# CederGroupHub/chgnet

Measured on NVIDIA H100. Metric: structures_per_sec_EFS, higher is better.
Workload: dtype f32

## Files before the change

chgnet_b200/_lib.py:

```python
from __future__ import annotations

import ctypes
import os
from ctypes import c_char_p, c_double, c_float, c_int32, c_int64, c_void_p

import torch
from torch import Tensor

_HERE = os.path.dirname(os.path.abspath(__file__))
LIB_PATH = os.path.join(_HERE, "libchgnet_b200.so")

P, I, F, D, I64 = c_void_p, c_int32, c_float, c_double, c_int64

SIGNATURES: dict[str, list] = {
    "chg_embed_atoms": [P, P, I, P, P],
    "chg_edge_geometry": [P, P, P, P, P, P, I, P, P, P, P],
    "chg_bond_basis_embed": [P, P, I, P, P, I, F, F, I, P, P, P, P, P, P],
    "chg_bond_basis_bwd": [P, P, I, P, P, I, F, F, I, P, P, P, P, P, P, P],
    "chg_angle_basis_embed": [P, P, P, I, P, I, P, P, P, P],
    "chg_angle_basis_bwd": [P, P, P, I, P, I, P, P, P, P, P],
    "chg_linear": [P, P, I, I, P, P, P, P, I, P, P],
    "chg_gather_rows": [P, P, I, I, P, P],
    "chg_scatter_rows": [P, P, I, I, P, P],
    "chg_atom_conv_fwd": [P, P, P, P, P, P, I, P, P, P, P, P, P, P],
    "chg_atom_conv_bwd": [P, P, P, P, P, P, I, P, P, P, P, P, P, P, P, P],
    "chg_segment_sum": [P, I, P, P, I, I, I, P, I, P],
    "chg_atom_conv_fused": [P, P, P, P, P, P, P, I, I, P, P, P, P, P, P, P],
    "chg_bond_conv_fused": [P, P, P, P, P, P, P, P, I, I, P, P, P, P, P, P, P, P],
    "chg_bond_conv_fwd": [P, P, P, P, P, P, P, I, P, P, P, P, P, P, P],
    "chg_bond_conv_bwd": [P, P, P, P, P, I, P, P, P, P, P, P, P, P, P],
    "chg_angle_update_fwd": [P, P, P, P, P, P, P, I, P, P, P, P],
    "chg_angle_update_bwd": [P, P, I, P, P, P, P],
    "chg_readout": [P, P, P, I, P, P, P, P, I, P, F, P, P, P, P, P, P, P],
    "chg_magmom": [P, I, P, F, P, P],
    "chg_force_virial": [P, P, P, P, P, P, P, P, P, P, I, P, P, P],
    "chg_wgrad": [P, P, I, P, I, P, I, P, I, I, P, I, P, P, P],
    "chg_colsum": [P, I, P, I, P, I, I, P, P],
    "chg_readout_bwd": [P, I, P, P, P, P, I, P, P, P, P, P, P, P, P],
    "chg_magmom_bwd": [P, I, P, F, P, P, P, P],
    "chg_loss_terms": [P, P, I, I, F, P, P, P],
    "chg_adam_step": [P, P, P, P, I64, F, F, F, F, F, I, P],
    "chg_edge_tangent": [P, P, P, P, P, P, P, P, I, P, P, P],
    "chg_bond_basis_tangent": [P, P, P, I, P, P, I, F, F, I, P, P, P, P, P, P],
    "chg_bond_basis_bwd2": [P, P, P, I, P, P, I, F, F, I, P, P, P, P, P, P],
    "chg_angle_basis_tangent": [P, P, P, P, I, P, I, P, P, P, P],
    "chg_angle_basis_bwd2": [P, P, P, P, I, P, I, P, P, P, P],
    "chg_atom_conv_tan": [P, P, P, P, P, P, P, I, P, P, P, P, P, P, P, P],
    "chg_atom_conv_bwd2": [P, P, P, P, P, P, P, P, P, I, P, P, P, P, P, P, P, P, P],
    "chg_bond_conv_tan": [P, P, P, P, P, P, P, P, I, P, P, P, P, P, P, P, P],
    "chg_bond_conv_bwd2": [P, P, P, P, P, P, P, P, P, I, P, P, P, P, P, P, P, P, P, P],
    "chg_angle_update_tan": [P, P, P, P, P, P, P, I, P, P, P, P, P],
    "chg_angle_update_bwd2": [P, P, P, P, I, P, P, P, P],
    "chg_readout_bwd2": [P, P, I, P, P, P, P, I, P, P, P, P, P, P, P, P, P, P, P, P],
    "chg_bond_basis_hvp": [P, P, P, I, P, P, I, F, F, I, P, P, P, P, P, P],
    "chg_angle_basis_hvp": [P, P, P, P, I, P, I, P, P, P, P],
    "chg_edge_tangent_bwd": [P, P, P, P, P, P, P, P, P, P, I, P, P],
    "chg_edge_tangent_bwd_virial": [P, P, P, P, P, P, P, P, P, P, P, P, I, P, P, P],
    "chg_dynamical_matrices": [P, P, P, P, P, I, I, P, I, P, P],
    "chg_dynamical_matrix_derivatives": [P, P, P, P, P, I, I, P, I, P, P, P],
# ... 141 lines not shown

    def atom_conv_bwd(self, pcn, pe, wag, center, nbr, d2u, save_p, g_agg, w2, ln, g_pre, g_w, g_p=None, g_ln=None):
        self._chk(pcn, pe, wag, center, nbr, d2u, save_p, g_agg, w2, ln, g_pre, g_w, g_p, g_ln)
        self._call("chg_atom_conv_bwd", _p(pcn), _p(pe), _p(wag), _p(center), _p(nbr), _p(d2u), center.shape[0],
                   _p(save_p), _p(g_agg), _p(w2), _p(ln), _p(g_pre), _p(g_w), _p(g_p), _p(g_ln))

    def _fused_work(self, n_rows: int, device) -> Tensor:
        need = int(self.lib.chg_gated_fused_workspace_floats(int(n_rows)))
        ws = getattr(self, "_fws", None)
        if ws is None or ws.device != device or ws.numel() < need:
            ws = torch.empty(need, dtype=torch.float32, device=device)
            self._fws = ws
        return ws

    def atom_conv_fused(self, pcn, pe, wag, center, nbr, d2u, ptr_c, w2t, b2, ln, agg, save_p):
        self._chk(pcn, pe, wag, center, nbr, d2u, ptr_c, w2t, b2, ln, agg, save_p)
        self._call("chg_atom_conv_fused", _p(pcn), _p(pe), _p(wag), _p(center), _p(nbr), _p(d2u), _p(ptr_c), center.shape[0],
                   agg.shape[0], _p(w2t), _p(b2), _p(ln), _p(agg), _p(save_p), _p(self._fused_work(center.shape[0], agg.device)))

    def bond_conv_fused(self, pij, px, pa, wbg, ang_atom, ang_i, ang_j, ptr_i, w2t, b2, ln, agg, save_pre, save_p):
        self._chk(pij, px, pa, wbg, ang_atom, ang_i, ang_j, ptr_i, w2t, b2, ln, agg, save_pre, save_p)
        self._call("chg_bond_conv_fused", _p(pij), _p(px), _p(pa), _p(wbg), _p(ang_atom), _p(ang_i), _p(ang_j), _p(ptr_i),
                   ang_i.shape[0], agg.shape[0], _p(w2t), _p(b2), _p(ln), _p(agg), _p(save_pre), _p(save_p),
                   _p(self._fused_work(ang_i.shape[0], agg.device)))

    def segment_sum(self, data, perm, ptr, accumulate, out):
        self._chk(data, perm, ptr)
        if not out.is_cuda or out.stride(1) != 1:
            raise ChgnetB200Error("segment_sum output must be a CUDA tensor with unit column stride")
        n_items = data.shape[0] if perm is None else perm.shape[0]
        self._call("chg_segment_sum", _p(data), data.shape[1], _p(perm), _p(ptr), ptr.shape[0] - 1, n_items,
                   int(accumulate), _p(out), out.stride(0))

    def bond_conv_fwd(self, pij, px, pa, wbg, ang_atom, ang_i, ang_j, w2t, b2, ln, upd, save_pre, save_p):
        self._chk(pij, px, pa, wbg, ang_atom, ang_i, ang_j, w2t, b2, ln, upd, save_pre, save_p)
        self._call("chg_bond_conv_fwd", _p(pij), _p(px), _p(pa), _p(wbg), _p(ang_atom), _p(ang_i), _p(ang_j),
                   ang_i.shape[0], _p(w2t), _p(b2), _p(ln), _p(upd), _p(save_pre), _p(save_p))

    def bond_conv_bwd(self, save_pre, save_p, wbg, ang_i, ang_j, g_agg, w2, ln, g_pre, gw_i, gw_j, g_p=None,
                      g_ln=None):
        self._chk(save_pre, save_p, wbg, ang_i, ang_j, g_agg, w2, ln, g_pre, gw_i, gw_j, g_p, g_ln)
        self._call("chg_bond_conv_bwd", _p(save_pre), _p(save_p), _p(wbg), _p(ang_i), _p(ang_j), ang_i.shape[0],
                   _p(g_agg), _p(w2), _p(ln), _p(g_pre), _p(gw_i), _p(gw_j), _p(g_p), _p(g_ln))

    def angle_update_fwd(self, pij, px, pa, ang, ang_atom, ang_i, ang_j, ln, ang_new, save_p):
        self._chk(pij, px, pa, ang, ang_atom, ang_i, ang_j, ln, ang_new, save_p)
        self._call("chg_angle_update_fwd", _p(pij), _p(px), _p(pa), _p(ang), _p(ang_atom), _p(ang_i), _p(ang_j),
                   ang_i.shape[0], _p(ln), _p(ang_new), _p(save_p))

    def angle_update_bwd(self, save_p, g_ang_in, ln, g_pre, g_ln=None):
        self._chk(save_p, g_ang_in, ln, g_pre, g_ln)
        self._call("chg_angle_update_bwd", _p(save_p), _p(g_ang_in), save_p.shape[0], _p(ln), _p(g_pre), _p(g_ln))

    @staticmethod
    def _chk_rows(*tensors: Tensor | None) -> None:
        for t in tensors:
            if t is not None and (not t.is_cuda or t.stride(-1) != 1):
                raise ChgnetB200Error("kernel arguments must be CUDA tensors with unit column stride")

    def _workspace(self, n_out: int, device) -> Tensor:
        ws = getattr(self, "_ws", None)
        if ws is None or ws.device != device:
            need = max(int(self.lib.chg_wgrad_workspace_floats(n)) for n in (64, 128, 256))
            ws = torch.empty(need, dtype=torch.float32, device=device)
            self._ws = ws
        return ws
# ... 225 lines not shown
```

chgnet_b200/csrc/common.cuh:

```cuda
#pragma once
#include <cuda_runtime.h>
#include <stdint.h>

#include "../../include/chgnet_b200.h"

namespace chg {

void set_error(const char* fmt, ...);
void count_launch();
int sm_count();
int linear_impl();
int gated_impl();
int segsum_unroll();
int segsum_force_s();

#define CHG_CHECK_ARG(cond, msg)                \
  do {                                          \
    if (!(cond)) {                              \
      chg::set_error("%s: %s", __func__, msg);  \
      return CHG_ERR_ARG;                       \
    }                                           \
  } while (0)

#define CHG_CUDA(expr)                                                              \
  do {                                                                              \
    cudaError_t _e = (expr);                                                        \
    if (_e != cudaSuccess) {                                                        \
      chg::set_error("%s: %s failed: %s", __func__, #expr, cudaGetErrorString(_e)); \
      return CHG_ERR_CUDA;                                                          \
    }                                                                               \
  } while (0)

#define CHG_LAUNCH_END()                                                            \
  do {                                                                              \
    cudaError_t _e = cudaGetLastError();                                            \
    if (_e != cudaSuccess) {                                                        \
      chg::set_error("%s: launch failed: %s", __func__, cudaGetErrorString(_e));    \
      return CHG_ERR_CUDA;                                                          \
    }                                                                               \
    chg::count_launch();                                                            \
    return CHG_OK;                                                                  \
  } while (0)

static inline cudaStream_t as_stream(void* s) { return reinterpret_cast<cudaStream_t>(s); }

#ifdef __CUDACC__

// ... 53 lines not shown
```

chgnet_b200/csrc/linear_ws.cu:

```cuda
#include <cuda.h>

#include "common.cuh"
#include "tc.cuh"

namespace chg {
namespace {

constexpr int NTHR = 288;
constexpr int PRODUCER_WARP = 8;
constexpr int S_IN = 2;
constexpr int PANEL = 128 * 128;
constexpr int IN_STAGE = 2 * PANEL;

struct Bars {
  uint64_t in_full[S_IN], in_empty[S_IN];
  uint64_t res_full, out_empty;
};

__device__ __forceinline__ void tma_load_2d(void* smem_dst, const CUtensorMap* map, int c0, int c1, uint64_t* bar) {
  asm volatile(
      "cp.async.bulk.tensor.2d.shared::cluster.global.mbarrier::complete_tx::bytes [%0], [%1, {%3, %4}], [%2];" ::"r"(
          tc::smem_u32(smem_dst)),
      "l"(map), "r"(tc::smem_u32(bar)), "r"(c0), "r"(c1)
      : "memory");
}
__device__ __forceinline__ void tma_store_2d(const CUtensorMap* map, int c0, int c1, const void* smem_src) {
  asm volatile("cp.async.bulk.tensor.2d.global.shared::cta.bulk_group [%0, {%2, %3}], [%1];" ::"l"(map),
               "r"(tc::smem_u32(smem_src)), "r"(c0), "r"(c1)
               : "memory");
}
__device__ __forceinline__ int swz(int r, int c) { return r * 128 + ((c ^ (r & 7)) << 4); }
__device__ __forceinline__ int panel_offset(int r, int col) { return (col >> 5) * PANEL + swz(r, (col & 31) >> 2) + (col & 3) * 4; }

template <int NT>
__global__ void __launch_bounds__(NTHR, 1)
linear_ws_kernel(const __grid_constant__ CUtensorMap map_x, const __grid_constant__ CUtensorMap map_y,
                 const __grid_constant__ CUtensorMap map_r, int m, int k, const float* __restrict__ wt,
                 const float* __restrict__ bias, int has_residual, int n_out) {
  extern __shared__ __align__(1024) uint8_t smem_raw[];
  uint8_t* s_in = smem_raw + ((1024u - (tc::smem_u32(smem_raw) & 1023u)) & 1023u);
  uint8_t* s_out = s_in + S_IN * IN_STAGE;
  uint8_t* s_bhi = s_out + (NT / 32) * PANEL;
  uint8_t* s_blo = s_bhi + (size_t)NT * k * 4;
  __shared__ __align__(8) Bars bars;
  __shared__ __align__(16) float s_bias[NT];

  const int tid = threadIdx.x, warp = tid >> 5, lane = tid & 31;
  const int col_base = blockIdx.y * NT;
  const int n_tiles = (m + 127) / 128;
  const int k_chunks = k / 64;

  {
    const int n4 = NT / 4, total4 = n4 * k;
    for (int i4 = tid; i4 < total4; i4 += NTHR) {
      const int kk = i4 / n4, n0 = (i4 % n4) * 4;
      const float4 v = ldg4(wt + (size_t)kk * n_out + col_base + n0);
#pragma unroll
      for (int e = 0; e < 4; ++e) {
        uint32_t hi, lo;
        tc::split_tf32(f4at(v, e), hi, lo);
        const uint32_t off = tc::kmajor_offset(n0 + e, kk, k);
        *reinterpret_cast<uint32_t*>(s_bhi + off) = hi;
        *reinterpret_cast<uint32_t*>(s_blo + off) = lo;
      }
    }
  }
  if (tid < NT) s_bias[tid] = bias != nullptr ? bias[col_base + tid] : 0.f;
  if (tid == 0) {
    for (int i = 0; i < S_IN; ++i) {
      tc::mbar_init(&bars.in_full[i], 1);
      tc::mbar_init(&bars.in_empty[i], 256);
    }
    tc::mbar_init(&bars.res_full, 1);
    tc::mbar_init(&bars.out_empty, 1);
    tc::mbar_fence_init();
  }
  tc::fence_async_smem();
  __syncthreads();

  if (warp == PRODUCER_WARP) {
    if (lane == 0) {
      int it = 0, tile_it = 0;
      for (int tile = blockIdx.x; tile < n_tiles; tile += gridDim.x, ++tile_it) {
        const int base = tile * 128;
        for (int kc = 0; kc < k_chunks; ++kc, ++it) {
          const int s = it % S_IN;
          tc::mbar_wait(&bars.in_empty[s], ((it / S_IN) & 1) ^ 1);
          tc::mbar_expect_tx(&bars.in_full[s], IN_STAGE);
          tma_load_2d(s_in + s * IN_STAGE, &map_x, kc * 64, base, &bars.in_full[s]);
          tma_load_2d(s_in + s * IN_STAGE + PANEL, &map_x, kc * 64 + 32, base, &bars.in_full[s]);
        }
        if (has_residual) {
          tc::mbar_wait(&bars.out_empty, (tile_it & 1) ^ 1);
          tc::mbar_expect_tx(&bars.res_full, (uint32_t)(NT / 32) * PANEL);
#pragma unroll
          for (int p = 0; p < NT / 32; ++p) tma_load_2d(s_out + p * PANEL, &map_r, col_base + p * 32, base, &bars.res_full);
        }
      }
    }
  } else {
    const int t = tid;
    const int row0 = (warp >> 2) * 64;
    const uint32_t bhi_addr = tc::smem_u32(s_bhi), blo_addr = tc::smem_u32(s_blo);
    const uint32_t sbo = (uint32_t)(k / 4) * 128;
    int it = 0, tile_it = 0;
    for (int tile = blockIdx.x; tile < n_tiles; tile += gridDim.x, ++tile_it) {
      const int base = tile * 128;
      float acc[NT / 2];
#pragma unroll
      for (int i = 0; i < NT / 2; ++i) acc[i] = 0.f;
      for (int kc = 0; kc < k_chunks; ++kc, ++it) {
        const int s = it % S_IN;
        tc::mbar_wait(&bars.in_full[s], (it / S_IN) & 1);
        const uint8_t* stage = s_in + s * IN_STAGE;
        tc::wg_gemm_k64<NT>(acc, [&](int r, int kk) { return *reinterpret_cast<const float*>(stage + panel_offset(row0 + r, kk)); },
                            bhi_addr + kc * 2048, blo_addr + kc * 2048, sbo);
        tc::mbar_arrive(&bars.in_empty[s]);
      }
      if (has_residual) tc::mbar_wait(&bars.res_full, tile_it & 1);
      tc::wg_barrier(2, 256);
#pragma unroll
      for (int i = 0; i < NT / 2; i += 2) {
        const int r = row0 + tc::frag_row(i), col = tc::frag_col(i);
        float2* dst = reinterpret_cast<float2*>(s_out + panel_offset(r, col));
        float2 o = make_float2(acc[i] + s_bias[col], acc[i + 1] + s_bias[col + 1]);
        if (has_residual) {
          const float2 res = *dst;
          o.x += res.x;
          o.y += res.y;
        }
        *dst = o;
      }
      tc::fence_async_smem();
// ... 10 lines not shown
  }
}

typedef CUresult (*EncodeFn)(CUtensorMap*, CUtensorMapDataType, cuuint32_t, void*, const cuuint64_t*,
                             const cuuint64_t*, const cuuint32_t*, const cuuint32_t*, CUtensorMapInterleave,
                             CUtensorMapSwizzle, CUtensorMapL2promotion, CUtensorMapFloatOOBfill);

EncodeFn encode_fn() {
  static EncodeFn fn = nullptr;
  static bool tried = false;
  if (!tried) {
    tried = true;
    void* p = nullptr;
    cudaDriverEntryPointQueryResult qres;
    if (cudaGetDriverEntryPoint("cuTensorMapEncodeTiled", &p, cudaEnableDefault, &qres) == cudaSuccess &&
        qres == cudaDriverEntryPointSuccess)
      fn = reinterpret_cast<EncodeFn>(p);
  }
  return fn;
}

bool make_map(CUtensorMap* map, const float* ptr, int rows, int cols) {
  EncodeFn fn = encode_fn();
  if (fn == nullptr) return false;
  const cuuint64_t dims[2] = {(cuuint64_t)cols, (cuuint64_t)rows};
  const cuuint64_t strides[1] = {(cuuint64_t)cols * 4};
  const cuuint32_t box[2] = {32, 128};
  const cuuint32_t estr[2] = {1, 1};
  return fn(map, CU_TENSOR_MAP_DATA_TYPE_FLOAT32, 2, const_cast<float*>(ptr), dims, strides, box, estr,
            CU_TENSOR_MAP_INTERLEAVE_NONE, CU_TENSOR_MAP_SWIZZLE_128B, CU_TENSOR_MAP_L2_PROMOTION_L2_128B,
            CU_TENSOR_MAP_FLOAT_OOB_FILL_NONE) == CUDA_SUCCESS;
}

template <int NT>
int launch_ws(const CUtensorMap& mx, const CUtensorMap& my, const CUtensorMap& mr, int m, int k, const float* wt,
              const float* bias, int has_residual, int n_out, cudaStream_t stream) {
  const int smem = S_IN * IN_STAGE + (NT / 32) * PANEL + 2 * NT * k * 4 + 1024;
  static int max_smem_set = 0;
  if (smem > max_smem_set) {
    CHG_CUDA(cudaFuncSetAttribute(linear_ws_kernel<NT>, cudaFuncAttributeMaxDynamicSharedMemorySize, smem));
    max_smem_set = smem;
  }
  const int n_tiles = (m + 127) / 128;
  const int col_tiles = n_out / NT;
  dim3 grid(min(n_tiles, max(1, sm_count() / col_tiles)), col_tiles);
  linear_ws_kernel<NT><<<grid, NTHR, smem, stream>>>(mx, my, mr, m, k, wt, bias, has_residual, n_out);
  CHG_LAUNCH_END();
}

}

int linear_ws(const float* x, int m, int k, const float* wt, const float* bias, const float* residual, int n_out,
              float* y, cudaStream_t stream) {
  if (k != 64 && k != 128) return 1;
  CUtensorMap mx, my, mr;
  if (!make_map(&mx, x, m, k) || !make_map(&my, y, m, n_out)) return 1;
  if (residual != nullptr) {
    if (!make_map(&mr, residual, m, n_out)) return 1;
  } else {
    mr = my;
  }
  if (n_out % 128 == 0 && k == 64) return launch_ws<128>(mx, my, mr, m, k, wt, bias, residual != nullptr, n_out, stream);
  return launch_ws<64>(mx, my, mr, m, k, wt, bias, residual != nullptr, n_out, stream);
}

}
```

chgnet_b200/csrc/native_engine.cu:

```cuda
#include <cstdarg>
#include <cstdio>
#include <cstring>
#include <string>

#include "common.cuh"

namespace chg {
namespace {

constexpr size_t ALIGN = 256;
constexpr int64_t PAD = 16;

struct GatedW {
  const float *w2t = nullptr, *w2 = nullptr, *b2 = nullptr, *ln = nullptr;
  const float *a_t = nullptr, *b_t = nullptr, *c_t = nullptr, *bias1 = nullptr;
  const float *a_b = nullptr, *b_b = nullptr, *c_b = nullptr;
  const float *wo_t = nullptr, *wo = nullptr, *bo = nullptr;
};
struct Weights {
  const float *emb, *freq_ag, *freq_bg, *freq_ang, *w3t, *w3, *wang_t, *wang;
  GatedW atom[CHG_MAX_CONV], bond[CHG_MAX_CONV], angle[CHG_MAX_CONV];
  const float *readout_ln, *mlp_wt, *mlp_w, *mlp_b, *w_last, *w_mag, *atom_ref;
};

// ... 251 lines not shown
    float* xn = c.f(true, (size_t)N * 64);
    atom_conv(n_conv - 1, x, xn);
    x = xn;
  }

  float* h_out = o.crystal_fea != nullptr ? c.f(false, (size_t)N * 64) : nullptr;
  float* g_x = grad ? c.f(true, (size_t)N * 64) : nullptr;
  c.zero(o.energy, (size_t)B * 8);
  c.zero(o.e_ref, (size_t)B * 8);
  RUN(c, "readout", chg_readout(x, b.z, b.owner, N, W.readout_ln, W.mlp_wt, W.mlp_w, W.mlp_b, hp.n_readout_hidden, W.w_last,
                                hp.b_last, W.atom_ref, o.site_e, h_out, o.energy, o.e_ref, g_x, st));
  if (o.crystal_fea != nullptr) seg(h_out, 64, nullptr, b.graph_ptr, B, N, 0, o.crystal_fea, 64);
  c.ar.reset_tmp();
  if (!grad) return c.rc;

  float* g_e = c.f(true, (size_t)Eu * 64);
  bool g_e_live = false;
  float* g_wag = c.f(true, (size_t)Eu * 64);
  c.zero(g_wag, (size_t)Eu * 256);
  float* g_wbg = has_ang ? c.f(true, (size_t)Es * 64) : nullptr;
  if (has_ang) c.zero(g_wbg, (size_t)Es * 256);
  float* g_a = has_ang ? c.f(true, (size_t)A * 64) : nullptr;
  bool g_a_live = false;

  auto atom_bwd = [&](int t) {
    const GatedW& g = W.atom[t];
    float* g_agg = c.f(false, (size_t)N * 64);
    lin(g_x, nullptr, N, 64, g.wo, nullptr, nullptr, nullptr, 64, g_agg);
    float* g_pre = c.f(false, (size_t)Ed * 128);
    float* g_w = c.f(false, (size_t)Ed * 64);
    RUN(c, "atom_conv_bwd", chg_atom_conv_bwd(sa[t].pcn, sa[t].pe, wag, b.center, b.nbr, b.d2u, Ed, sa[t].p, g_agg, g.w2, g.ln,
                                              g_pre, g_w, nullptr, nullptr, st));
    float* sp = c.f(false, (size_t)N * 256);
    seg(g_pre, 128, nullptr, b.ptr_c, N, Ed, 0, sp, 256);
    seg(g_pre, 128, b.perm_n, b.ptr_n, N, Ed, 0, sp + 128, 256);
    lin(sp, nullptr, N, 256, g.a_b, nullptr, g_x, nullptr, 64, g_x);
    float* spe = c.f(false, (size_t)Eu * 128);
    seg(g_pre, 128, b.perm_u, b.ptr_u, Eu, Ed, 0, spe, 128);
    lin(spe, nullptr, Eu, 128, g.b_b, nullptr, g_e_live ? g_e : nullptr, nullptr, 64, g_e);
    g_e_live = true;
    seg(g_w, 64, b.perm_u, b.ptr_u, Eu, Ed, 1, g_wag, 64);
    c.ar.reset_tmp();
  };
  auto angle_scatter = [&](const float* g_pre, const GatedW& g) {
    float* sp = c.f(false, (size_t)Es * 256);
    seg(g_pre, 128, nullptr, b.ptr_is, Es, A, 0, sp, 256);
    seg(g_pre, 128, b.perm_js, b.ptr_js, Es, A, 0, sp + 128, 256);
    lin(sp, nullptr, Es, 256, g.a_b, nullptr, g_e, b.short_ids, 64, g_e);
    float* spx = c.f(false, (size_t)N * 128);
    seg(g_pre, 128, b.perm_x, b.ptr_x, N, A, 0, spx, 128);
    lin(spx, nullptr, N, 128, g.b_b, nullptr, g_x, nullptr, 64, g_x);
  };

  atom_bwd(n_conv - 1);
  for (int t = n_conv - 2; t >= 0; --t) {
    if (has_ang) {
      if (t < n_conv - 2) {
        const GatedW& ga = W.angle[t];
        float* g_pre = c.f(false, (size_t)A * 128);
        RUN(c, "angle_update_bwd", chg_angle_update_bwd(sang[t], g_a_live ? g_a : nullptr, A, ga.ln, g_pre, nullptr, st));
        lin(g_pre, nullptr, A, 128, ga.c_b, nullptr, g_a_live ? g_a : nullptr, nullptr, 64, g_a);
        g_a_live = true;
        angle_scatter(g_pre, ga);
        c.ar.reset_tmp();
      }
      const GatedW& g = W.bond[t];
      float* g_agg = c.f(false, (size_t)Es * 64);
      lin(g_e, b.short_ids, Es, 64, g.wo, nullptr, nullptr, nullptr, 64, g_agg);
      float* g_pre = c.f(false, (size_t)A * 128);
      float *gw_i = c.f(false, (size_t)A * 64), *gw_j = c.f(false, (size_t)A * 64);
      RUN(c, "bond_conv_bwd", chg_bond_conv_bwd(sb[t].pre, sb[t].p, wbg_s, b.ang_is, b.ang_js, A, g_agg, g.w2, g.ln, g_pre, gw_i,
                                                gw_j, nullptr, nullptr, st));
      lin(g_pre, nullptr, A, 128, g.c_b, nullptr, g_a_live ? g_a : nullptr, nullptr, 64, g_a);
      g_a_live = true;
      angle_scatter(g_pre, g);
      seg(gw_i, 64, nullptr, b.ptr_is, Es, A, 1, g_wbg, 64);
      seg(gw_j, 64, b.perm_js, b.ptr_js, Es, A, 1, g_wbg, 64);
      c.ar.reset_tmp();
    }
    atom_bwd(t);
  }

  float* g_dist = c.f(false, Eu);
  float* g_wbg_full = c.f(false, (size_t)Eu * 64);
  c.zero(g_wbg_full, (size_t)Eu * 256);
  if (has_ang) RUN(c, "scatter_rows", chg_scatter_rows(g_wbg, b.short_ids, Es, 64, g_wbg_full, st));
  RUN(c, "bond_basis_bwd", chg_bond_basis_bwd(dist, b.u2d, Eu, W.freq_ag, W.freq_bg, hp.num_radial, hp.atom_graph_cutoff,
                                              hp.bond_graph_cutoff, hp.cutoff_coeff, W.w3, g_e, g_wag, g_wbg_full, g_dist, nullptr, st));
  double* g_rhat = static_cast<double*>(c.ar.tmp((size_t)Ed * 3 * 8));
  c.zero(g_rhat, (size_t)Ed * 24);
  if (has_ang)
    RUN(c, "angle_basis_bwd", chg_angle_basis_bwd(rhat, b.ang_di, b.ang_dj, A, W.freq_ang, (hp.num_angular - 1) / 2, W.wang, g_a,
                                                  g_rhat, nullptr, st));
  c.zero(o.force, (size_t)N * 24);
  c.zero(o.virial, (size_t)B * 72);
  RUN(c, "force_virial", chg_force_virial(rvec, dist, rhat, g_rhat, g_dist, b.d2u, b.u2d, b.center, b.nbr, b.owner, Ed, o.force,
                                          o.virial, st));
  c.ar.reset_tmp();
  return c.rc;
}

}
}

using namespace chg;

extern "C" int64_t chg_packed_floats(const chg_hparams* hp) {
// ... 135 lines not shown
```

chgnet_b200/csrc/segsum.cu:

```cuda
#include "common.cuh"

namespace chg {
namespace {

template <int W, int S, int U>
__global__ void __launch_bounds__(256)
segment_sum_kernel(const float* __restrict__ data, const int32_t* __restrict__ perm,
                   const int32_t* __restrict__ ptr, int n_rows, int accumulate, float* out, int out_ld) {
  constexpr int LANES = W / 4;
  constexpr int GROUPS = 256 / LANES;
  constexpr int ROWS = GROUPS / S;
  __shared__ float4 s_part[S > 1 ? 256 : 1];
  const int sub = threadIdx.x % LANES;
  const int grp = threadIdx.x / LANES;
  const int row_in_cta = grp / S, split = grp % S;
  const int n_pass = (n_rows + ROWS - 1) / ROWS;
  for (int pass = blockIdx.x; pass < n_pass; pass += gridDim.x) {
    const int r = pass * ROWS + row_in_cta;
    float4 a0 = make_float4(0.f, 0.f, 0.f, 0.f), a1 = a0, a2 = a0, a3 = a0;
    if (r < n_rows) {
      const int beg = ptr[r] + split, end = ptr[r + 1];
      const float* base = data + (size_t)sub * 4;
      int k = beg;
      if (perm == nullptr) {
// ... 44 lines not shown
          const float4 v3 = ldg4(base + (size_t)i3 * W);
          a0 = a0 + v0; a1 = a1 + v1; a2 = a2 + v2; a3 = a3 + v3;
        }
        for (; k < end; k += S) a0 = a0 + ldg4(base + (size_t)perm[k] * W);
      }
    }
    float4 s = (a0 + a1) + (a2 + a3);
    if (S > 1) {
      s_part[threadIdx.x] = s;
      __syncthreads();
      if (split == 0) {
#pragma unroll
        for (int j = 1; j < S; ++j) s = s + s_part[threadIdx.x + j * LANES];
      }
      __syncthreads();
    }
    if (split == 0 && r < n_rows) {
      float* dst = out + (size_t)r * out_ld + sub * 4;
      if (accumulate) s = s + *reinterpret_cast<const float4*>(dst);
      stg4(dst, s);
    }
  }
}

template <int W, int S, int U>
void launch_segsum(const float* data, const int32_t* perm, const int32_t* ptr, int n_rows, int accumulate,
                   float* out, int out_ld, cudaStream_t stream) {
  constexpr int ROWS = (256 / (W / 4)) / S;
  const int n_pass = (n_rows + ROWS - 1) / ROWS;
  const int blocks = max(1, min(n_pass, sm_count() * 8));
  segment_sum_kernel<W, S, U><<<blocks, 256, 0, stream>>>(data, perm, ptr, n_rows, accumulate, out, out_ld);
}

template <bool SCATTER>
__global__ void move_rows_kernel(const float* __restrict__ src, const int32_t* __restrict__ idx, int n, int width,
                                 float* __restrict__ dst) {
  const int per_row = width / 4;
  const long long t = (long long)blockIdx.x * blockDim.x + threadIdx.x;
  if (t >= (long long)n * per_row) return;
  const int i = (int)(t / per_row), c4 = (int)(t % per_row);
  const int j = idx[i];
  const size_t s_row = SCATTER ? (size_t)i : (size_t)j, d_row = SCATTER ? (size_t)j : (size_t)i;
  stg4(dst + d_row * width + c4 * 4, ldg4(src + s_row * width + c4 * 4));
}

}
}

using namespace chg;

extern "C" int chg_gather_rows(const float* src, const int32_t* idx, int32_t n, int32_t width, float* dst,
                               void* stream) {
  CHG_CHECK_ARG(n >= 0 && width > 0 && width % 4 == 0, "bad size");
  if (n == 0) return CHG_OK;
  CHG_CHECK_ARG(src && idx && dst, "null pointer");
  const long long total = (long long)n * (width / 4);
  move_rows_kernel<false><<<(unsigned)((total + 255) / 256), 256, 0, as_stream(stream)>>>(src, idx, n, width, dst);
  CHG_LAUNCH_END();
}

extern "C" int chg_scatter_rows(const float* src, const int32_t* idx, int32_t n, int32_t width, float* dst,
                                void* stream) {
  CHG_CHECK_ARG(n >= 0 && width > 0 && width % 4 == 0, "bad size");
  if (n == 0) return CHG_OK;
  CHG_CHECK_ARG(src && idx && dst, "null pointer");
  const long long total = (long long)n * (width / 4);
  move_rows_kernel<true><<<(unsigned)((total + 255) / 256), 256, 0, as_stream(stream)>>>(src, idx, n, width, dst);
  CHG_LAUNCH_END();
}

extern "C" int chg_segment_sum(const float* data, int32_t width, const int32_t* perm, const int32_t* ptr,
                               int32_t n_rows, int32_t n_items, int32_t accumulate, float* out, int32_t out_ld,
                               void* stream) {
  CHG_CHECK_ARG(n_rows >= 0 && n_items >= 0, "negative size");
  CHG_CHECK_ARG(width == 64 || width == 128, "width must be 64 or 128");
  CHG_CHECK_ARG(out_ld >= width && out_ld % 4 == 0, "out_ld must be >= width and a multiple of 4");
  if (n_rows == 0) return CHG_OK;
  CHG_CHECK_ARG(ptr && out, "null pointer");
  const int avg = n_items / n_rows;
  const int groups = 256 / (width / 4);
  const int resident = sm_count() * 8;
  int S = 1;
  while (S < 8 && avg >= 16 * S && ((long long)n_rows * (2 * S) + groups - 1) / groups <= resident) S *= 2;
  if (S == 1 && avg >= 32) S = 2;
  if (segsum_force_s() > 0) S = segsum_force_s();
  const bool u8 = segsum_unroll() == 8;
  cudaStream_t st = as_stream(stream);
#define CHG_SEG(W_, S_)                                                              \
  do {                                                                               \
    if (u8) launch_segsum<W_, S_, 8>(data, perm, ptr, n_rows, accumulate, out, out_ld, st); \
    else launch_segsum<W_, S_, 4>(data, perm, ptr, n_rows, accumulate, out, out_ld, st);    \
  } while (0)
  if (width == 64) {
    if (S == 1) CHG_SEG(64, 1); else if (S == 2) CHG_SEG(64, 2); else if (S == 4) CHG_SEG(64, 4); else CHG_SEG(64, 8);
  } else {
    if (S == 1) CHG_SEG(128, 1); else if (S == 2) CHG_SEG(128, 2); else if (S == 4) CHG_SEG(128, 4); else CHG_SEG(128, 8);
  }
#undef CHG_SEG
  CHG_LAUNCH_END();
}
```

include/chgnet_b200.h:

```cpp
#ifndef CHGNET_B200_H
#define CHGNET_B200_H

#include <stdint.h>

#ifdef __cplusplus
extern "C" {
#endif

#define CHG_FEA 64
#define CHG_MAX_CONV 8
#define CHG_MAX_Z 94
#define CHG_OK 0
#define CHG_ERR_ARG (-1)
#define CHG_ERR_CUDA (-2)

const char* chg_last_error(void);
int chg_abi_version(void);
int64_t chg_launch_count(void);
int chg_set_option(const char* name, int32_t value);

int chg_embed_atoms(const int32_t* z, const float* emb, int32_t n_atoms, float* x, void* stream);

int chg_edge_geometry(const float* frac, const float* lattice, const int32_t* atom_owner,
                      const int32_t* center, const int32_t* nbr, const float* image,
// ... 17 lines not shown
                          int32_t n_angles, const float* freq, int32_t n_freq,
                          const float* wt, float* a0,
                          float* basis_out ,
                          void* stream);
int chg_angle_basis_bwd(const float* rhat, const int32_t* ang_di, const int32_t* ang_dj,
                        int32_t n_angles, const float* freq, int32_t n_freq,
                        const float* w, const float* g_a0, double* g_rhat ,
                        double* g_freq , void* stream);

int chg_linear(const float* x, const int32_t* x_rows, int32_t m, int32_t k, const float* wt,
               const float* bias, const float* residual, const int32_t* y_rows, int32_t n_out,
               float* y, void* stream);
int chg_gather_rows(const float* src, const int32_t* idx, int32_t n, int32_t width, float* dst,
                    void* stream);
int chg_scatter_rows(const float* src, const int32_t* idx, int32_t n, int32_t width, float* dst,
                     void* stream);

int chg_atom_conv_fwd(const float* pcn, const float* pe, const float* wag,
                      const int32_t* center, const int32_t* nbr, const int32_t* d2u,
                      int32_t n_edges, const float* w2t, const float* b2, const float* ln,
                      float* msg, float* save_p, float* save_pre ,
                      void* stream);
int chg_atom_conv_bwd(const float* pcn, const float* pe, const float* wag,
                      const int32_t* center, const int32_t* nbr, const int32_t* d2u,
                      int32_t n_edges, const float* save_p, const float* g_agg,
                      const float* w2, const float* ln, float* g_pre, float* g_w,
                      float* g_p ,
                      double* g_ln , void* stream);

int chg_segment_sum(const float* data, int32_t width, const int32_t* perm,
                    const int32_t* ptr, int32_t n_rows,
                    int32_t n_items , int32_t accumulate,
                    float* out, int32_t out_ld , void* stream);

int64_t chg_gated_fused_workspace_floats(int32_t n_rows);
int chg_atom_conv_fused(const float* pcn, const float* pe, const float* wag, const int32_t* center,
                        const int32_t* nbr, const int32_t* d2u, const int32_t* ptr_c, int32_t n_edges,
                        int32_t n_atoms, const float* w2t, const float* b2, const float* ln, float* agg,
                        float* save_p, float* work, void* stream);
int chg_bond_conv_fused(const float* pij, const float* px, const float* pa, const float* wbg,
                        const int32_t* ang_atom, const int32_t* ang_i, const int32_t* ang_j,
                        const int32_t* ptr_i, int32_t n_angles, int32_t n_slots, const float* w2t,
                        const float* b2, const float* ln, float* agg, float* save_pre, float* save_p,
                        float* work, void* stream);

int chg_bond_conv_fwd(const float* pij, const float* px, const float* pa, const float* wbg,
                      const int32_t* ang_atom, const int32_t* ang_i, const int32_t* ang_j,
                      int32_t n_angles, const float* w2t, const float* b2, const float* ln,
                      float* upd, float* save_pre, float* save_p, void* stream);
int chg_bond_conv_bwd(const float* save_pre, const float* save_p, const float* wbg,
                      const int32_t* ang_i, const int32_t* ang_j, int32_t n_angles,
                      const float* g_agg, const float* w2, const float* ln, float* g_pre,
                      float* gw_i, float* gw_j, float* g_p ,
                      double* g_ln , void* stream);

int chg_angle_update_fwd(const float* pij, const float* px, const float* pa, const float* ang,
                         const int32_t* ang_atom, const int32_t* ang_i, const int32_t* ang_j,
                         int32_t n_angles, const float* ln, float* ang_new, float* save_p,
                         void* stream);
int chg_angle_update_bwd(const float* save_p, const float* g_ang_in, int32_t n_angles,
                         const float* ln, float* g_pre, double* g_ln ,
                         void* stream);

int chg_readout(const float* x, const int32_t* z, const int32_t* atom_owner, int32_t n_atoms,
                const float* ln, const float* mlp_wt, const float* mlp_w, const float* mlp_b,
                int32_t n_hidden, const float* w_last, float b_last, const float* atom_ref,
// ... 229 lines not shown
```

Before: 10880.

## Fuse backward edge segment sums and angle projection with scatter

Replaces four separate segment-sum launches in the atom-conv backward with one edge-pair kernel. That kernel reads each g_pre row once and produces the per-atom center/neighbor sums, the per-bond pair sums and the g_wag accumulation together. In the angle backward, the g_pre→g_a linear is fused with the ptr_is segment sum: extra warps in the warp-specialized TMA linear kernel reduce segments from the shared-memory input tiles, and a small kernel handles segments that cross tiles. The aim is to cut launches and repeated global reads of g_pre, at the cost of more complex code, an assumption of exactly two directed edges per bond, and extra threads in the linear kernel.

```diff
diff --git a/chgnet_b200/_lib.py b/chgnet_b200/_lib.py
--- a/chgnet_b200/_lib.py
+++ b/chgnet_b200/_lib.py
@@ -25,6 +25,8 @@
     "chg_atom_conv_fwd": [P, P, P, P, P, P, I, P, P, P, P, P, P, P],
     "chg_atom_conv_bwd": [P, P, P, P, P, P, I, P, P, P, P, P, P, P, P, P],
     "chg_segment_sum": [P, I, P, P, I, I, I, P, I, P],
+    "chg_edge_pair_scatter": [P, P, P, P, P, P, P, I, I, I, P, P, P, P],
+    "chg_angle_project_scatter": [P, P, P, I, I, P, P, P, P, I, P],
     "chg_atom_conv_fused": [P, P, P, P, P, P, P, I, I, P, P, P, P, P, P, P],
     "chg_bond_conv_fused": [P, P, P, P, P, P, P, P, I, I, P, P, P, P, P, P, P, P],
     "chg_bond_conv_fwd": [P, P, P, P, P, P, P, I, P, P, P, P, P, P, P],
@@ -232,6 +234,18 @@
         self._call("chg_segment_sum", _p(data), data.shape[1], _p(perm), _p(ptr), ptr.shape[0] - 1, n_items,
                    int(accumulate), _p(out), out.stride(0))
 
+    def edge_pair_scatter(self, g_pre, g_w, ptr_c, perm_n, d2u, perm_u, ptr_u, sp, spe, g_wag):
+        self._chk(g_pre, g_w, ptr_c, perm_n, d2u, perm_u, ptr_u, sp, spe, g_wag)
+        self._call("chg_edge_pair_scatter", _p(g_pre), _p(g_w), _p(ptr_c), _p(perm_n), _p(d2u), _p(perm_u), _p(ptr_u),
+                   ptr_c.shape[0] - 1, d2u.shape[0], ptr_u.shape[0] - 1, _p(sp), _p(spe), _p(g_wag))
+
+    def angle_project_scatter(self, g_pre, ang_is, ptr_is, w1a_b, residual, g_a, sp):
+        self._chk(g_pre, ang_is, ptr_is, w1a_b, residual, g_a)
+        if not sp.is_cuda or sp.stride(1) != 1:
+            raise ChgnetB200Error("angle_project_scatter sp must be a CUDA tensor with unit column stride")
+        self._call("chg_angle_project_scatter", _p(g_pre), _p(ang_is), _p(ptr_is), g_pre.shape[0], ptr_is.shape[0] - 1,
+                   _p(w1a_b), _p(residual), _p(g_a), _p(sp), sp.stride(0))
+
     def bond_conv_fwd(self, pij, px, pa, wbg, ang_atom, ang_i, ang_j, w2t, b2, ln, upd, save_pre, save_p):
         self._chk(pij, px, pa, wbg, ang_atom, ang_i, ang_j, w2t, b2, ln, upd, save_pre, save_p)
         self._call("chg_bond_conv_fwd", _p(pij), _p(px), _p(pa), _p(wbg), _p(ang_atom), _p(ang_i), _p(ang_j),
diff --git a/chgnet_b200/csrc/common.cuh b/chgnet_b200/csrc/common.cuh
--- a/chgnet_b200/csrc/common.cuh
+++ b/chgnet_b200/csrc/common.cuh
@@ -13,6 +13,7 @@
 int gated_impl();
 int segsum_unroll();
 int segsum_force_s();
+int segsum_splits(int n_rows, int n_items, int width);
 
 #define CHG_CHECK_ARG(cond, msg)                \
   do {                                          \
diff --git a/chgnet_b200/csrc/linear_ws.cu b/chgnet_b200/csrc/linear_ws.cu
--- a/chgnet_b200/csrc/linear_ws.cu
+++ b/chgnet_b200/csrc/linear_ws.cu
@@ -4,18 +4,50 @@
 #include "tc.cuh"
 
 namespace chg {
+
+__device__ __forceinline__ float2 operator+(const float2& a, const float2& b) { return make_float2(a.x + b.x, a.y + b.y); }
+
 namespace {
 
 constexpr int NTHR = 288;
+constexpr int NTHR_SCATTER = NTHR + 128;
 constexpr int PRODUCER_WARP = 8;
 constexpr int S_IN = 2;
 constexpr int PANEL = 128 * 128;
 constexpr int IN_STAGE = 2 * PANEL;
+constexpr int STRIP = 16;
 
 struct Bars {
   uint64_t in_full[S_IN], in_empty[S_IN];
   uint64_t res_full, out_empty;
 };
+
+struct SegArgs {
+  const int32_t* seg;
+  const int32_t* ptr;
+  float* out;
+  int out_ld;
+  int splits;
+};
+
+template <typename V, typename Row>
+__device__ __forceinline__ V seg_sum_ordered(int beg, int end, int splits, Row row) {
+  V total;
+  for (int j = 0; j < splits; ++j) {
+    V a0 = V{}, a1 = V{}, a2 = V{}, a3 = V{};
+    int k = beg + j;
+    for (; k + 3 * splits < end; k += 4 * splits) {
+      a0 = a0 + row(k);
+      a1 = a1 + row(k + splits);
+      a2 = a2 + row(k + 2 * splits);
+      a3 = a3 + row(k + 3 * splits);
+    }
+    for (; k < end; k += splits) a0 = a0 + row(k);
+    const V sj = (a0 + a1) + (a2 + a3);
+    total = j == 0 ? sj : total + sj;
+  }
+  return total;
+}
 
 __device__ __forceinline__ void tma_load_2d(void* smem_dst, const CUtensorMap* map, int c0, int c1, uint64_t* bar) {
   asm volatile(
@@ -32,11 +64,11 @@
 __device__ __forceinline__ int swz(int r, int c) { return r * 128 + ((c ^ (r & 7)) << 4); }
 __device__ __forceinline__ int panel_offset(int r, int col) { return (col >> 5) * PANEL + swz(r, (col & 31) >> 2) + (col & 3) * 4; }
 
-template <int NT>
-__global__ void __launch_bounds__(NTHR, 1)
+template <int NT, bool SCATTER>
+__global__ void __launch_bounds__(SCATTER ? NTHR_SCATTER : NTHR, 1)
 linear_ws_kernel(const __grid_constant__ CUtensorMap map_x, const __grid_constant__ CUtensorMap map_y,
                  const __grid_constant__ CUtensorMap map_r, int m, int k, const float* __restrict__ wt,
-                 const float* __restrict__ bias, int has_residual, int n_out) {
+                 const float* __restrict__ bias, int has_residual, int n_out, const SegArgs sa) {
   extern __shared__ __align__(1024) uint8_t smem_raw[];
   uint8_t* s_in = smem_raw + ((1024u - (tc::smem_u32(smem_raw) & 1023u)) & 1023u);
   uint8_t* s_out = s_in + S_IN * IN_STAGE;
@@ -52,7 +84,7 @@
 
   {
     const int n4 = NT / 4, total4 = n4 * k;
-    for (int i4 = tid; i4 < total4; i4 += NTHR) {
+    for (int i4 = tid; i4 < total4; i4 += (int)blockDim.x) {
       const int kk = i4 / n4, n0 = (i4 % n4) * 4;
       const float4 v = ldg4(wt + (size_t)kk * n_out + col_base + n0);
 #pragma unroll
@@ -69,7 +101,7 @@
   if (tid == 0) {
     for (int i = 0; i < S_IN; ++i) {
       tc::mbar_init(&bars.in_full[i], 1);
-      tc::mbar_init(&bars.in_empty[i], 256);
+      tc::mbar_init(&bars.in_empty[i], SCATTER ? 256 + 128 : 256);
     }
     tc::mbar_init(&bars.res_full, 1);
     tc::mbar_init(&bars.out_empty, 1);
@@ -98,7 +130,42 @@
         }
       }
     }
-  } else {
+  } else if (SCATTER && warp > PRODUCER_WARP) {
+    const int rw = warp - PRODUCER_WARP - 1;
+    auto tile_row = [&](int tile) { return tile * 128 + (rw + 4 * (lane >> 4)) * STRIP + (lane & 15); };
+    auto begins_at = [&](int tile, int& seg) {
+      const int row = tile_row(tile);
+      if (tile >= n_tiles || row >= m) return false;
+      seg = __ldg(sa.seg + row);
+      return row == 0 || __ldg(sa.seg + row - 1) != seg;
+    };
+    int nxt_seg = 0;
+    bool nxt_begins = begins_at(blockIdx.x, nxt_seg);
+    int nxt_end = nxt_begins ? __ldg(sa.ptr + nxt_seg + 1) : 0;
+    int it = 0;
+    for (int tile = blockIdx.x; tile < n_tiles; tile += gridDim.x) {
+      const int base = tile * 128;
+      const int my_seg = nxt_seg, my_end = nxt_end;
+      const unsigned own = __ballot_sync(0xffffffffu, nxt_begins && my_end <= base + 128);
+      nxt_begins = begins_at(tile + gridDim.x, nxt_seg);
+      for (int kc = 0; kc < k_chunks; ++kc, ++it) {
+        const int s = it % S_IN;
+        tc::mbar_wait(&bars.in_full[s], (it / S_IN) & 1);
+        const uint8_t* stage = s_in + s * IN_STAGE;
+        for (unsigned todo = own; todo != 0; todo &= todo - 1) {
+          const int i = __ffs(todo) - 1;
+          const int seg = __shfl_sync(0xffffffffu, my_seg, i), end = __shfl_sync(0xffffffffu, my_end, i);
+          const int beg = base + (rw + 4 * (i >> 4)) * STRIP + (i & 15);
+          const float2 v = seg_sum_ordered<float2>(beg, end, sa.splits, [&](int r) {
+            return *reinterpret_cast<const float2*>(stage + panel_offset(r - base, lane * 2));
+          });
+          *reinterpret_cast<float2*>(sa.out + (size_t)seg * sa.out_ld + kc * 64 + lane * 2) = v;
+        }
+        tc::mbar_arrive(&bars.in_empty[s]);
+      }
+      nxt_end = nxt_begins ? __ldg(sa.ptr + nxt_seg + 1) : 0;
+    }
+  } else if (warp < PRODUCER_WARP) {
     const int t = tid;
     const int row0 = (warp >> 2) * 64;
     const uint32_t bhi_addr = tc::smem_u32(s_bhi), blo_addr = tc::smem_u32(s_blo);
@@ -175,19 +242,20 @@
             CU_TENSOR_MAP_FLOAT_OOB_FILL_NONE) == CUDA_SUCCESS;
 }
 
-template <int NT>
+template <int NT, bool SCATTER = false>
 int launch_ws(const CUtensorMap& mx, const CUtensorMap& my, const CUtensorMap& mr, int m, int k, const float* wt,
-              const float* bias, int has_residual, int n_out, cudaStream_t stream) {
+              const float* bias, int has_residual, int n_out, cudaStream_t stream, const SegArgs& sa = SegArgs{}) {
   const int smem = S_IN * IN_STAGE + (NT / 32) * PANEL + 2 * NT * k * 4 + 1024;
   static int max_smem_set = 0;
   if (smem > max_smem_set) {
-    CHG_CUDA(cudaFuncSetAttribute(linear_ws_kernel<NT>, cudaFuncAttributeMaxDynamicSharedMemorySize, smem));
+    CHG_CUDA(cudaFuncSetAttribute(linear_ws_kernel<NT, SCATTER>, cudaFuncAttributeMaxDynamicSharedMemorySize, smem));
     max_smem_set = smem;
   }
   const int n_tiles = (m + 127) / 128;
   const int col_tiles = n_out / NT;
   dim3 grid(min(n_tiles, max(1, sm_count() / col_tiles)), col_tiles);
-  linear_ws_kernel<NT><<<grid, NTHR, smem, stream>>>(mx, my, mr, m, k, wt, bias, has_residual, n_out);
+  linear_ws_kernel<NT, SCATTER><<<grid, SCATTER ? NTHR_SCATTER : NTHR, smem, stream>>>(mx, my, mr, m, k, wt, bias,
+                                                                                       has_residual, n_out, sa);
   CHG_LAUNCH_END();
 }
 
@@ -207,4 +275,46 @@
   return launch_ws<64>(mx, my, mr, m, k, wt, bias, residual != nullptr, n_out, stream);
 }
 
-}
+namespace {
+
+__global__ void seg_cross_kernel(const float* __restrict__ x, const int32_t* __restrict__ ptr, int n_seg, int splits,
+                                 float* __restrict__ out, int out_ld) {
+  const int s = (int)((blockIdx.x * (size_t)blockDim.x + threadIdx.x) >> 5), lane = threadIdx.x & 31;
+  if (s >= n_seg) return;
+  const int beg = ptr[s], end = ptr[s + 1];
+  if (beg < end && beg / 128 == (end - 1) / 128) return;
+  const float4 v = seg_sum_ordered<float4>(beg, end, splits, [&](int r) { return ldg4(x + (size_t)r * 128 + lane * 4); });
+  stg4(out + (size_t)s * out_ld + lane * 4, v);
+}
+
+}
+
+}
+
+using namespace chg;
+
+extern "C" int chg_angle_project_scatter(const float* g_pre, const int32_t* ang_is, const int32_t* ptr_is,
+                                         int32_t n_angles, int32_t n_slots, const float* w1a_b, const float* residual,
+                                         float* g_a, float* sp, int32_t sp_ld, void* stream) {
+  CHG_CHECK_ARG(n_angles >= 0 && n_slots >= 0, "negative size");
+  CHG_CHECK_ARG(sp_ld >= 128 && sp_ld % 4 == 0, "sp_ld must be >= 128 and a multiple of 4");
+  if (n_slots == 0 && n_angles == 0) return CHG_OK;
+  CHG_CHECK_ARG(ptr_is && sp, "null pointer");
+  cudaStream_t st = as_stream(stream);
+  const int splits = segsum_splits(n_slots, n_angles, 128);
+  if (n_angles > 0) {
+    CHG_CHECK_ARG(g_pre && ang_is && w1a_b && g_a && n_slots > 0, "null pointer");
+    CUtensorMap mx, my, mr;
+    if (!make_map(&mx, g_pre, n_angles, 128) || !make_map(&my, g_a, n_angles, 64) ||
+        (residual != nullptr && !make_map(&mr, residual, n_angles, 64))) {
+      set_error("chg_angle_project_scatter: cuTensorMapEncodeTiled failed");
+      return CHG_ERR_CUDA;
+    }
+    if (residual == nullptr) mr = my;
+    const int rc = launch_ws<64, true>(mx, my, mr, n_angles, 128, w1a_b, nullptr, residual != nullptr, 64, st,
+                                       SegArgs{ang_is, ptr_is, sp, sp_ld, splits});
+    if (rc != CHG_OK) return rc;
+  }
+  seg_cross_kernel<<<(n_slots + 7) / 8, 256, 0, st>>>(g_pre, ptr_is, n_slots, splits, sp, sp_ld);
+  CHG_LAUNCH_END();
+}
diff --git a/chgnet_b200/csrc/native_engine.cu b/chgnet_b200/csrc/native_engine.cu
--- a/chgnet_b200/csrc/native_engine.cu
+++ b/chgnet_b200/csrc/native_engine.cu
@@ -307,19 +307,23 @@
     RUN(c, "atom_conv_bwd", chg_atom_conv_bwd(sa[t].pcn, sa[t].pe, wag, b.center, b.nbr, b.d2u, Ed, sa[t].p, g_agg, g.w2, g.ln,
                                               g_pre, g_w, nullptr, nullptr, st));
     float* sp = c.f(false, (size_t)N * 256);
-    seg(g_pre, 128, nullptr, b.ptr_c, N, Ed, 0, sp, 256);
-    seg(g_pre, 128, b.perm_n, b.ptr_n, N, Ed, 0, sp + 128, 256);
+    float* spe = c.f(false, (size_t)Eu * 128);
+    c.go("segment_sum");
+    if (c.go("segment_sum"))
+      c.rc = chg_edge_pair_scatter(g_pre, g_w, b.ptr_c, b.perm_n, b.d2u, b.perm_u, b.ptr_u, N, Ed, Eu, sp, spe, g_wag, st);
     lin(sp, nullptr, N, 256, g.a_b, nullptr, g_x, nullptr, 64, g_x);
-    float* spe = c.f(false, (size_t)Eu * 128);
-    seg(g_pre, 128, b.perm_u, b.ptr_u, Eu, Ed, 0, spe, 128);
+    c.go("segment_sum");
     lin(spe, nullptr, Eu, 128, g.b_b, nullptr, g_e_live ? g_e : nullptr, nullptr, 64, g_e);
     g_e_live = true;
-    seg(g_w, 64, b.perm_u, b.ptr_u, Eu, Ed, 1, g_wag, 64);
+    c.go("segment_sum");
     c.ar.reset_tmp();
   };
   auto angle_scatter = [&](const float* g_pre, const GatedW& g) {
     float* sp = c.f(false, (size_t)Es * 256);
-    seg(g_pre, 128, nullptr, b.ptr_is, Es, A, 0, sp, 256);
+    c.go("linear");
+    if (c.go("segment_sum"))
+      c.rc = chg_angle_project_scatter(g_pre, b.ang_is, b.ptr_is, A, Es, g.c_b, g_a_live ? g_a : nullptr, g_a, sp, 256, st);
+    g_a_live = true;
     seg(g_pre, 128, b.perm_js, b.ptr_js, Es, A, 0, sp + 128, 256);
     lin(sp, nullptr, Es, 256, g.a_b, nullptr, g_e, b.short_ids, 64, g_e);
     float* spx = c.f(false, (size_t)N * 128);
@@ -334,8 +338,6 @@
         const GatedW& ga = W.angle[t];
         float* g_pre = c.f(false, (size_t)A * 128);
         RUN(c, "angle_update_bwd", chg_angle_update_bwd(sang[t], g_a_live ? g_a : nullptr, A, ga.ln, g_pre, nullptr, st));
-        lin(g_pre, nullptr, A, 128, ga.c_b, nullptr, g_a_live ? g_a : nullptr, nullptr, 64, g_a);
-        g_a_live = true;
         angle_scatter(g_pre, ga);
         c.ar.reset_tmp();
       }
@@ -346,8 +348,6 @@
       float *gw_i = c.f(false, (size_t)A * 64), *gw_j = c.f(false, (size_t)A * 64);
       RUN(c, "bond_conv_bwd", chg_bond_conv_bwd(sb[t].pre, sb[t].p, wbg_s, b.ang_is, b.ang_js, A, g_agg, g.w2, g.ln, g_pre, gw_i,
                                                 gw_j, nullptr, nullptr, st));
-      lin(g_pre, nullptr, A, 128, g.c_b, nullptr, g_a_live ? g_a : nullptr, nullptr, 64, g_a);
-      g_a_live = true;
       angle_scatter(g_pre, g);
       seg(gw_i, 64, nullptr, b.ptr_is, Es, A, 1, g_wbg, 64);
       seg(gw_j, 64, b.perm_js, b.ptr_js, Es, A, 1, g_wbg, 64);
diff --git a/chgnet_b200/csrc/segsum.cu b/chgnet_b200/csrc/segsum.cu
--- a/chgnet_b200/csrc/segsum.cu
+++ b/chgnet_b200/csrc/segsum.cu
@@ -100,6 +100,106 @@
   segment_sum_kernel<W, S, U><<<blocks, 256, 0, stream>>>(data, perm, ptr, n_rows, accumulate, out, out_ld);
 }
 
+}
+
+int segsum_splits(int n_rows, int n_items, int width) {
+  const int avg = n_items / n_rows;
+  const int groups = 256 / (width / 4);
+  const int resident = sm_count() * 8;
+  int S = 1;
+  while (S < 8 && avg >= 16 * S && ((long long)n_rows * (2 * S) + groups - 1) / groups <= resident) S *= 2;
+  if (S == 1 && avg >= 32) S = 2;
+  if (segsum_force_s() > 0) S = segsum_force_s();
+  return S;
+}
+
+namespace {
+
+template <int S>
+__global__ void __launch_bounds__(256)
+edge_pair_scatter_kernel(const float* __restrict__ g_pre, const float* __restrict__ g_w, const int32_t* __restrict__ ptr_c,
+                         const int32_t* __restrict__ perm_n, const int32_t* __restrict__ d2u,
+                         const int32_t* __restrict__ perm_u, const int32_t* __restrict__ ptr_u, int n_atoms,
+                         float* __restrict__ sp, float* __restrict__ spe, float* __restrict__ g_wag) {
+  constexpr int ROWS = 8 / S;
+  __shared__ float4 s_part[S > 1 ? 2 * 256 : 1];
+  const int lane = threadIdx.x & 31, warp = threadIdx.x >> 5;
+  const int row_in_cta = warp / S, split = warp % S;
+  const int n_pass = (n_atoms + ROWS - 1) / ROWS;
+  const float* base = g_pre + lane * 4;
+  for (int pass = blockIdx.x; pass < n_pass; pass += gridDim.x) {
+    const int r = pass * ROWS + row_in_cta;
+    float4 a0 = make_float4(0.f, 0.f, 0.f, 0.f), a1 = a0, a2 = a0, a3 = a0, b0 = a0, b1 = a0, b2 = a0, b3 = a0;
+    if (r < n_atoms) {
+      const int end = ptr_c[r + 1];
+      auto row = [&](int e, int f, int rev, int u, bool first, float4& a, float4& b) {
+        const float4 v = ldg4(base + (size_t)e * 128), w = ldg4(base + (size_t)f * 128);
+        a = a + v;
+        b = b + w;
+        if (first) {
+          const float4 r = rev == f ? w : ldg4(base + (size_t)rev * 128);
+          stg4(spe + (size_t)u * 128 + lane * 4, v + r);
+          if (lane < 16) {
+            float4* dst = reinterpret_cast<float4*>(g_wag + (size_t)u * 64) + lane;
+            *dst = (ldg4(g_w + (size_t)e * 64 + lane * 4) + ldg4(g_w + (size_t)rev * 64 + lane * 4)) + *dst;
+          }
+        }
+      };
+      for (int k0 = ptr_c[r] + split; k0 < end; k0 += 32 * S) {
+        const int my_e = k0 + lane * S;
+        int my_f = 0, my_rev = 0, my_u = 0, my_first = 0;
+        if (my_e < end) {
+          my_f = perm_n[my_e];
+          my_u = d2u[my_e];
+          const int p = ptr_u[my_u];
+          const int e0 = perm_u[p], e1 = perm_u[p + 1];
+          my_first = e0 == my_e;
+          my_rev = my_first ? e1 : e0;
+        }
+        const int nb = min(32, (end - k0 + S - 1) / S);
+        int i = 0;
+        for (; i + 3 < nb; i += 4) {
+          const int f0 = __shfl_sync(0xffffffffu, my_f, i), f1 = __shfl_sync(0xffffffffu, my_f, i + 1);
+          const int f2 = __shfl_sync(0xffffffffu, my_f, i + 2), f3 = __shfl_sync(0xffffffffu, my_f, i + 3);
+          const int r0 = __shfl_sync(0xffffffffu, my_rev, i), r1 = __shfl_sync(0xffffffffu, my_rev, i + 1);
+          const int r2 = __shfl_sync(0xffffffffu, my_rev, i + 2), r3 = __shfl_sync(0xffffffffu, my_rev, i + 3);
+          const int u0 = __shfl_sync(0xffffffffu, my_u, i), u1 = __shfl_sync(0xffffffffu, my_u, i + 1);
+          const int u2 = __shfl_sync(0xffffffffu, my_u, i + 2), u3 = __shfl_sync(0xffffffffu, my_u, i + 3);
+          const unsigned first = __ballot_sync(0xffffffffu, my_first) >> i;
+          row(k0 + i * S, f0, r0, u0, first & 1u, a0, b0);
+          row(k0 + (i + 1) * S, f1, r1, u1, first & 2u, a1, b1);
+          row(k0 + (i + 2) * S, f2, r2, u2, first & 4u, a2, b2);
+          row(k0 + (i + 3) * S, f3, r3, u3, first & 8u, a3, b3);
+        }
+        for (; i < nb; ++i) {
+          const int f = __shfl_sync(0xffffffffu, my_f, i), rv = __shfl_sync(0xffffffffu, my_rev, i);
+          const int u = __shfl_sync(0xffffffffu, my_u, i);
+          const bool first = __shfl_sync(0xffffffffu, my_first, i) != 0;
+          row(k0 + i * S, f, rv, u, first, a0, b0);
+        }
+      }
+    }
+    float4 s = (a0 + a1) + (a2 + a3), t = (b0 + b1) + (b2 + b3);
+    if (S > 1) {
+      s_part[threadIdx.x] = s;
+      s_part[256 + threadIdx.x] = t;
+      __syncthreads();
+      if (split == 0) {
+#pragma unroll
+        for (int j = 1; j < S; ++j) {
+          s = s + s_part[threadIdx.x + j * 32];
+          t = t + s_part[256 + threadIdx.x + j * 32];
+        }
+      }
+      __syncthreads();
+    }
+    if (split == 0 && r < n_atoms) {
+      stg4(sp + (size_t)r * 256 + lane * 4, s);
+      stg4(sp + (size_t)r * 256 + 128 + lane * 4, t);
+    }
+  }
+}
+
 template <bool SCATTER>
 __global__ void move_rows_kernel(const float* __restrict__ src, const int32_t* __restrict__ idx, int n, int width,
                                  float* __restrict__ dst) {
@@ -145,13 +245,7 @@
   CHG_CHECK_ARG(out_ld >= width && out_ld % 4 == 0, "out_ld must be >= width and a multiple of 4");
   if (n_rows == 0) return CHG_OK;
   CHG_CHECK_ARG(ptr && out, "null pointer");
-  const int avg = n_items / n_rows;
-  const int groups = 256 / (width / 4);
-  const int resident = sm_count() * 8;
-  int S = 1;
-  while (S < 8 && avg >= 16 * S && ((long long)n_rows * (2 * S) + groups - 1) / groups <= resident) S *= 2;
-  if (S == 1 && avg >= 32) S = 2;
-  if (segsum_force_s() > 0) S = segsum_force_s();
+  const int S = segsum_splits(n_rows, n_items, width);
   const bool u8 = segsum_unroll() == 8;
   cudaStream_t st = as_stream(stream);
 #define CHG_SEG(W_, S_)                                                              \
@@ -167,3 +261,23 @@
 #undef CHG_SEG
   CHG_LAUNCH_END();
 }
+
+extern "C" int chg_edge_pair_scatter(const float* g_pre, const float* g_w, const int32_t* ptr_c, const int32_t* perm_n,
+                                     const int32_t* d2u, const int32_t* perm_u, const int32_t* ptr_u, int32_t n_atoms,
+                                     int32_t n_edges, int32_t n_bonds, float* sp, float* spe, float* g_wag, void* stream) {
+  CHG_CHECK_ARG(n_atoms >= 0 && n_edges >= 0 && n_bonds >= 0, "negative size");
+  CHG_CHECK_ARG(n_edges == 2 * n_bonds, "every bond must have exactly two directed edges");
+  if (n_atoms == 0) return CHG_OK;
+  CHG_CHECK_ARG(ptr_c && sp, "null pointer");
+  CHG_CHECK_ARG(n_edges == 0 || (g_pre && g_w && perm_n && d2u && perm_u && ptr_u && spe && g_wag), "null pointer");
+  const int S = segsum_splits(n_atoms, n_edges, 128);
+  const int rows = 8 / S;
+  const int blocks = max(1, min((n_atoms + rows - 1) / rows, sm_count() * 8));
+  cudaStream_t st = as_stream(stream);
+#define CHG_EPS(S_) \
+  edge_pair_scatter_kernel<S_><<<blocks, 256, 0, st>>>(g_pre, g_w, ptr_c, perm_n, d2u, perm_u, ptr_u, n_atoms, sp, spe, \
+                                                       g_wag)
+  if (S == 1) CHG_EPS(1); else if (S == 2) CHG_EPS(2); else if (S == 4) CHG_EPS(4); else CHG_EPS(8);
+#undef CHG_EPS
+  CHG_LAUNCH_END();
+}
diff --git a/include/chgnet_b200.h b/include/chgnet_b200.h
--- a/include/chgnet_b200.h
+++ b/include/chgnet_b200.h
@@ -73,6 +73,14 @@
                     const int32_t* ptr, int32_t n_rows,
                     int32_t n_items , int32_t accumulate,
                     float* out, int32_t out_ld , void* stream);
+
+int chg_edge_pair_scatter(const float* g_pre, const float* g_w, const int32_t* ptr_c, const int32_t* perm_n,
+                          const int32_t* d2u, const int32_t* perm_u, const int32_t* ptr_u, int32_t n_atoms,
+                          int32_t n_edges, int32_t n_bonds, float* sp, float* spe, float* g_wag, void* stream);
+
+int chg_angle_project_scatter(const float* g_pre, const int32_t* ang_is, const int32_t* ptr_is, int32_t n_angles,
+                              int32_t n_slots, const float* w1a_b, const float* residual, float* g_a, float* sp,
+                              int32_t sp_ld, void* stream);
 
 int64_t chg_gated_fused_workspace_floats(int32_t n_rows);
 int chg_atom_conv_fused(const float* pcn, const float* pe, const float* wag, const int32_t* center,
```

After: 11460, median of 6. 5.3% higher.
